# elvis-sik/muscle_synergies

Measured on NVIDIA B200. Metric: vicon_csv_loader_throughput, higher is better.
Workload: dtype f64

## Files before the change

include/ms_b200.h:

```cpp
#ifndef MS_B200_H
#define MS_B200_H

#include <stdint.h>

#ifdef __cplusplus
extern "C" {
#endif

#define MS_OK 0
#define MS_E_INVALID (-1)
#define MS_E_CUDA (-2)
#define MS_E_WORKSPACE (-3)
#define MS_E_NO_DEVICE (-4)

#ifndef MS_TILE_BYTES
#define MS_TILE_BYTES 49152
#endif
#define MS_MAX_ROW_BYTES 8192
#define MS_MAX_BLANK_ROWS 8
#define MS_MAX_SECTIONS 4

#define MS_SCAN_HAS_HIGH_BYTES 1u
#define MS_SCAN_BLANK_OVERFLOW 2u
#define MS_SCAN_HAS_CR 4u
// ... 105 lines not shown
    int64_t* d_stops;
    int64_t* d_offsets;
} ms_window_plan;
int ms_segment_trial(const double* d_left_fz, const double* d_right_fz, int64_t n, int32_t min_phase_size,
                     int32_t num_segments, void* d_work, int64_t* d_transitions, int32_t* d_loaded, int32_t* d_n_found,
                     const ms_window_plan* h_plans, int32_t n_plans, void* stream);

int ms_plan_phase_windows(const int64_t* d_transitions, const int32_t* d_n_found, int32_t num_segments,
                          int32_t cycles, int64_t divisor, int64_t n_rows, int32_t n_channels, int64_t* d_starts,
                          int64_t* d_stops, int64_t* d_offsets, void* stream);

int ms_cut_windows(const double* d_src, int64_t src_stride, int32_t n_channels, const int64_t* d_starts,
                   const int64_t* d_stops, const int64_t* d_out_offsets, int32_t n_windows, double* d_out,
                   int64_t max_window_len, void* stream);


int ms_channel_means(const double* d_src, int64_t stride, int32_t n_channels, int64_t n, double* d_mean, void* stream);
int ms_rms_envelope(const double* d_src, int64_t stride, int32_t n_channels, int64_t n, const double* d_mean,
                    int32_t window, double* d_out, int64_t out_stride, void* stream);
size_t ms_sosfilt_workspace_bytes(int64_t n, int32_t n_channels, int64_t padlen, int32_t zero_lag);
int ms_sosfilt(const double* d_src, int64_t stride, int32_t n_channels, int64_t n, const double* h_sos,
               int32_t n_sections, const double* h_zi, int64_t padlen, int32_t zero_lag, const double* d_mean,
               int32_t rectify, double* d_out, int64_t out_stride, void* d_work, void* stream);
int ms_time_normalize_windows(const double* d_env, int64_t stride, int32_t n_channels, const int64_t* d_starts,
                              const int64_t* d_stops, int32_t n_windows, int32_t reduce_to, int32_t normalize,
                              double* d_out, void* stream);


int32_t ms_nmf_resident_max_rows(int32_t m, int32_t kmax);
int ms_nmf_mu_batched(const float* d_X, int32_t n, int32_t m, const int32_t* h_ranks, const int32_t* h_x_index,
// ... 48 lines not shown
```

muscle_synergies_b200/_native.py:

```python
import ctypes
import os

_HERE = os.path.dirname(os.path.abspath(__file__))
LIB_PATH = os.path.join(_HERE, "libms_b200.so")

MS_TILE_BYTES = 49152
MS_MAX_ROW_BYTES = 8192
MS_MAX_BLANK_ROWS = 8
MS_MAX_SECTIONS = 4

MS_SCAN_HAS_HIGH_BYTES = 1
MS_SCAN_BLANK_OVERFLOW = 2
MS_SCAN_HAS_CR = 4

MS_ERR_NONE = 0xFFFFFFFFFFFFFFFF
MS_ERR_KIND_BAD_FLOAT = 1
MS_ERR_KIND_NON_ASCII = 2
MS_ERR_KIND_ROW_TOO_LONG = 3


class ScanSummary(ctypes.Structure):
    _fields_ = [
        ("n_bytes", ctypes.c_int64),
        ("n_rows", ctypes.c_int64),
# ... 57 lines not shown


class WindowPlan(ctypes.Structure):
    _fields_ = [
        ("divisor", ctypes.c_int64),
        ("n_rows", ctypes.c_int64),
        ("n_channels", ctypes.c_int32),
        ("cycles", ctypes.c_int32),
        ("d_starts", ctypes.c_void_p),
        ("d_stops", ctypes.c_void_p),
        ("d_offsets", ctypes.c_void_p),
    ]


MS_MAX_WINDOW_PLANS = 4


class NativeError(RuntimeError):
    pass


_lib = None


def _declare(L):
    vp, i64, i32 = ctypes.c_void_p, ctypes.c_int64, ctypes.c_int32
    sigs = {
        "ms_workspace_bytes": (i64, [i64]),
        "ms_workspace_masks_offset": (i64, [i64]),
        "ms_scan": (ctypes.c_int, [vp, i64, vp, i64, vp, vp]),
        "ms_scan_quoted": (ctypes.c_int, [vp, i64, vp, i64, vp, vp]),
        "ms_peek_after_blank": (ctypes.c_int, [vp, i64, vp, i32, vp, i32, vp, vp]),
        "ms_parse": (ctypes.c_int, [vp, i64, vp, ctypes.POINTER(Section), i32, vp, vp]),
        "ms_transitions_workspace_bytes": (i64, [i64]),
        "ms_find_transitions": (ctypes.c_int, [vp, vp, i64, i32, i32, vp, vp, vp, vp, vp]),
        "ms_segment_trial": (ctypes.c_int, [vp, vp, i64, i32, i32, vp, vp, vp, vp, ctypes.POINTER(WindowPlan), i32, vp]),
        "ms_cut_windows": (ctypes.c_int, [vp, i64, i32, vp, vp, vp, i32, vp, i64, vp]),
        "ms_plan_phase_windows": (ctypes.c_int, [vp, vp, i32, i32, i64, i64, i32, vp, vp, vp, vp]),
        "ms_channel_means": (ctypes.c_int, [vp, i64, i32, i64, vp, vp]),
        "ms_rms_envelope": (ctypes.c_int, [vp, i64, i32, i64, vp, i32, vp, i64, vp]),
        "ms_sosfilt_workspace_bytes": (ctypes.c_size_t, [i64, i32, i64, i32]),
        "ms_sosfilt": (ctypes.c_int, [vp, i64, i32, i64, ctypes.POINTER(ctypes.c_double), i32,
                                      ctypes.POINTER(ctypes.c_double), i64, i32, vp, i32, vp, i64, vp, vp]),
        "ms_time_normalize_windows": (ctypes.c_int, [vp, i64, i32, vp, vp, i32, i32, i32, vp, vp]),
        "ms_nmf_resident_max_rows": (i32, [i32, i32]),
        "ms_nmf_mu_batched": (ctypes.c_int, [vp, i32, i32, ctypes.POINTER(i32), ctypes.POINTER(i32), i32, vp, vp, i32,
                                             ctypes.c_float, i32, vp, vp, vp, vp, vp]),
        "ms_host_copy_stream": (ctypes.c_int, [vp, vp, i64]),
        "ms_nmf_plan": (i32, [i32, i32, ctypes.POINTER(i32), ctypes.POINTER(i32), i32, vp]),
        "ms_nmf_mu_batched_planned": (ctypes.c_int, [vp, i32, i32, vp, i32, i32, vp, vp, i32, ctypes.c_float, i32, vp, vp, vp, vp]),
        "ms_nmf_stream_workspace_bytes": (i64, [i32, i32]),
        "ms_nmf_mu_stream": (ctypes.c_int, [vp, i64, i32, ctypes.POINTER(i32), ctypes.POINTER(i32), i32, vp, vp, i32,
# ... 73 lines not shown
```

muscle_synergies_b200/csrc/ms_common.cuh:

```cuda
#pragma once
#include <cuda_runtime.h>
#include <stdint.h>

#include "../../include/ms_b200.h"

extern int64_t g_ms_launches;
extern thread_local char g_ms_last_error[256];

#define MS_CUDA_CHECK(expr)                                                                    \
    do {                                                                                       \
        cudaError_t _e = (expr);                                                               \
        if (_e != cudaSuccess) {                                                               \
            snprintf(g_ms_last_error, sizeof g_ms_last_error, "%s: %s", #expr, cudaGetErrorString(_e)); \
            return MS_E_CUDA;                                                                  \
        }                                                                                      \
    } while (0)

#define MS_COUNT_LAUNCH() ((void)__atomic_fetch_add(&g_ms_launches, 1, __ATOMIC_RELAXED))

__device__ __forceinline__ uint32_t ms_eq_flags(uint32_t w, uint32_t rep) {
    uint32_t y = w ^ rep;
    uint32_t t = (y & 0x7f7f7f7fu) + 0x7f7f7f7fu;
    return ~(t | y | 0x7f7f7f7fu);
}
// ... 50 lines not shown
```

muscle_synergies_b200/csrc/ms_fused.cu:

```cuda
#include <stdio.h>

#include "ms_field.cuh"

#ifndef FUSED_THREADS
#define FUSED_THREADS 512
#endif
#ifndef FUSED_AB_BASE
#ifndef FUSED_EARLY_COMMAS
#define FUSED_LATE_COMMAS
#endif
#define FUSED_WALK64
#define FUSED_PIN_LUT
#endif
#define FUSED_WARPS (FUSED_THREADS / 32)
#ifndef FUSED_MAX_TILE
#define FUSED_MAX_TILE MS_TILE_BYTES
#endif
#ifndef FUSED_MIN_CTAS
#define FUSED_MIN_CTAS 3
#endif
#define FUSED_MAX_REGION (FUSED_MAX_TILE + MS_MAX_ROW_BYTES)
#define FUSED_MAX_NSEG (FUSED_MAX_REGION / 16)
#define FUSED_PAD 16
#ifndef FUSED_LB_WINDOWS
// ... 933 lines not shown
static int ms_fused_tile_bytes(int32_t tile_bytes, int overhang) {
    const int largest = FUSED_MAX_REGION - overhang;
    if (tile_bytes <= 0) return largest;
    int t = tile_bytes / 16 * 16;
    if (t < 4096) t = 4096;
    if (t > largest) t = largest;
    return t;
}

extern "C" int64_t ms_load_workspace_bytes(int64_t n_bytes, int32_t tile_bytes) {
    (void)tile_bytes;
    const int64_t n_tiles = n_bytes <= 0 ? 0 : (n_bytes + 4095) / 4096;
    return FUSED_LB_OFFSET + (n_tiles + 1) * 8;
}

extern "C" int ms_load_fused(const uint8_t* d_bytes, int64_t n_bytes, const ms_load_plan* h_plan, void* d_workspace,
                             int64_t workspace_bytes, ms_load_result* d_result, uint8_t* d_peek, void* stream) {
    if (!d_bytes || !h_plan || !d_workspace || !d_result || !d_peek || n_bytes < 0) return MS_E_INVALID;
    if (((uintptr_t)d_bytes & 15) != 0 || ((uintptr_t)d_workspace & 15) != 0) return MS_E_INVALID;
    if (!h_plan->d_arena || h_plan->arena_elems < 0 || h_plan->cap_rows[0] <= 0 || h_plan->cap_rows[1] < 0) return MS_E_INVALID;
    const int overhang = ms_fused_overhang(h_plan->overhang_bytes);
    const int tile = ms_fused_tile_bytes(h_plan->tile_bytes, overhang);
    if (workspace_bytes < ms_load_workspace_bytes(n_bytes, tile)) return MS_E_WORKSPACE;
    cudaStream_t st = (cudaStream_t)stream;
    const int64_t need = FUSED_LB_OFFSET + ((n_bytes + tile - 1) / tile + 1) * 8;
    MS_CUDA_CHECK(cudaMemsetAsync(d_workspace, 0, (size_t)need, st));
    MS_CUDA_CHECK(cudaMemsetAsync(d_result, 0, sizeof(ms_load_result), st));
    MS_CUDA_CHECK(cudaMemsetAsync(&d_result->status, 0xFF, sizeof(uint64_t), st));
    const int64_t n_tiles = n_bytes == 0 ? 0 : (n_bytes + tile - 1) / tile;
    if (n_tiles == 0) return MS_OK;
// ... 16 lines not shown
```

muscle_synergies_b200/csrc/ms_segment.cu:

```cuda
#include <stdio.h>

#include <string.h>

#include "ms_common.cuh"

#define SEG_THREADS 1024
#define SEG_WARPS (SEG_THREADS / 32)
#define SEG_SPB 4
#define SEG_BLOCK_WORDS (32 * SEG_SPB)
static_assert(SEG_WARPS == 32, "a warp per bitmap word of a stretch");
#define SEG_MAX_HALO 2048

extern "C" int64_t ms_transitions_workspace_bytes(int64_t n) { return 2 * ((n + 31) / 32 + 2) * 4 + 16 + ((n + 1023) / 1024 + SEG_SPB) * 8; }

struct MsPlansArg {
    ms_window_plan p[MS_MAX_WINDOW_PLANS];
    int n;
};

__device__ void ms_plan_windows(const int64_t* __restrict__ transitions, int found, int num_segments, const ms_window_plan& pl) {
    const int per_trecho = pl.cycles ? 2 : 8, span = pl.cycles ? 4 : 1, n_windows = 4 * per_trecho;
    const bool ok = found >= num_segments && num_segments >= 40;
    int64_t off = 0;
    for (int w = 0; w < n_windows; w++) {
        int64_t a = 0, b = 0;
// ... 48 lines not shown
    if (e) {
        f = ((x >> (__ffs(e) - 1)) & 1u) ? 1u : 2u;
        l = ((x >> (31 - __clz(e))) & 1u) ? 1u : 2u;
    }
    uint32_t cy = f == 2u ? 1u : 0u;
    unsigned long long inc = seg_pack((unsigned long long)__popc(seg_changes(x, y, cy)), f, l);
#pragma unroll
    for (int d = 1; d < 32; d <<= 1) {
        const unsigned long long o = __shfl_up_sync(0xffffffffu, inc, d);
        if (lane >= d) inc = seg_combine(o, inc);
    }
    *inclusive = inc;
    return __shfl_sync(0xffffffffu, inc, 31);
}

__global__ void __launch_bounds__(SEG_THREADS, 2)
    ms_segment_kernel(const double* __restrict__ left, const double* __restrict__ right, int64_t n, int min_phase, int halo,
                      uint32_t* __restrict__ valid1, uint32_t* __restrict__ valid2, unsigned int* __restrict__ counter,
                      unsigned long long* __restrict__ summary, long long num_segments, int64_t* __restrict__ transitions,
                      int32_t* __restrict__ loaded, int32_t* __restrict__ n_found, const MsPlansArg plans) {
    extern __shared__ uint32_t s_r[];
    __shared__ bool s_last;
    __shared__ uint32_t s_v[2][SEG_BLOCK_WORDS];
    __shared__ unsigned long long s_scan[SEG_WARPS];
    __shared__ unsigned long long s_total;
    const int tid = threadIdx.x, lane = tid & 31, warp = tid >> 5;
    const int64_t n_words = (n + 31) / 32;
    const int64_t w_blk = (int64_t)blockIdx.x * SEG_BLOCK_WORDS;
    if (halo >= 0) {
        uint32_t* r1 = s_r;
        uint32_t* r2 = s_r + SEG_BLOCK_WORDS + halo;
        for (int wi0 = warp; wi0 < SEG_BLOCK_WORDS + halo; wi0 += SEG_WARPS * SEG_SPB) {
            double lv[SEG_SPB], rv[SEG_SPB];
#pragma unroll
            for (int q = 0; q < SEG_SPB; q++) {
                const int64_t i = (w_blk + wi0 + q * SEG_WARPS) * 32 + lane;
                const bool in = wi0 + q * SEG_WARPS < SEG_BLOCK_WORDS + halo && i < n;
                lv[q] = in ? left[i] : 0.0;
                rv[q] = in ? right[i] : 0.0;
            }
#pragma unroll
            for (int q = 0; q < SEG_SPB; q++) {
                const int wi = wi0 + q * SEG_WARPS;
                const int64_t i = (w_blk + wi) * 32 + lane;
                const bool a = lv[q] != 0.0, b = rv[q] != 0.0;
                const bool x1 = i < n ? a != b : true, x2 = i < n ? a && b : true;
                const uint32_t b1 = __ballot_sync(0xffffffffu, x1), b2 = __ballot_sync(0xffffffffu, x2);
                if (lane == 0 && wi < SEG_BLOCK_WORDS + halo) {
                    r1[wi] = b1;
                    r2[wi] = b2;
                }
            }
        }
        __syncthreads();
    }
#pragma unroll
    for (int q = 0; q < SEG_SPB; q++) {
        const int wl = warp + q * SEG_WARPS;
        const int64_t i_own = (w_blk + wl) * 32 + lane;
        bool v1 = false, v2 = false;
        if (i_own < n) {
            if (halo < 0) {
                const int64_t end = min(n, i_own + (int64_t)min_phase);
                v1 = v2 = true;
                for (int64_t j = i_own; j < end; j++) {
                    const bool a = left[j] != 0.0, b = right[j] != 0.0;
                    v1 = v1 && (a != b);
                    v2 = v2 && (a && b);
                    if (!v1 && !v2) break;
                }
            } else if (min_phase <= 0) {
                v1 = (s_r[wl] >> lane) & 1u;
                v2 = (s_r[SEG_BLOCK_WORDS + halo + wl] >> lane) & 1u;
            } else {
                v1 = ms_bits_all_set(s_r, wl, lane, min_phase);
                v2 = ms_bits_all_set(s_r + SEG_BLOCK_WORDS + halo, wl, lane, min_phase);
            }
        }
        const uint32_t w1 = __ballot_sync(0xffffffffu, v1), w2 = __ballot_sync(0xffffffffu, v2);
        if (lane == 0) {
            s_v[0][wl] = w1;
            s_v[1][wl] = w2;
            if (w_blk + wl < n_words) {
                valid1[w_blk + wl] = w1;
                valid2[w_blk + wl] = w2;
            }
        }
    }
    __syncthreads();
    if (warp < SEG_SPB) {
        unsigned long long inc;
        const unsigned long long total = seg_warp_scan(s_v[0][warp * 32 + lane], s_v[1][warp * 32 + lane], lane, &inc);
        if (lane == 0) summary[(int64_t)blockIdx.x * SEG_SPB + warp] = total;
    }
#if defined(SEG_ABLATE) && SEG_ABLATE == 1
    return;
#endif
    __threadfence();
    __syncthreads();
    if (tid == 0) s_last = atomicInc(counter, gridDim.x - 1) == gridDim.x - 1;
    __syncthreads();
    if (!s_last) return;
#if defined(SEG_ABLATE) && SEG_ABLATE == 2
    return;
#endif
    __threadfence();
    unsigned long long before = seg_pack(0, 2, 2);
    const int64_t n_blocks = (int64_t)gridDim.x * SEG_SPB;
    for (int64_t base = 0; base < n_blocks; base += SEG_THREADS) {
        const int64_t blk = base + tid;
        const unsigned long long mine = blk < n_blocks ? __ldcg(summary + blk) : 0ull;
        unsigned long long inc = mine;
#pragma unroll
        for (int d = 1; d < 32; d <<= 1) {
            const unsigned long long o = __shfl_up_sync(0xffffffffu, inc, d);
            if (lane >= d) inc = seg_combine(o, inc);
        }
        if (lane == 31) s_scan[warp] = inc;
        __syncthreads();
        if (warp == 0) {
            unsigned long long v = s_scan[lane];
#pragma unroll
            for (int d = 1; d < 32; d <<= 1) {
                const unsigned long long o = __shfl_up_sync(0xffffffffu, v, d);
                if (lane >= d) v = seg_combine(o, v);
            }
            s_scan[lane] = v;
            if (lane == 31) s_total = seg_combine(before, v);
        }
        __syncthreads();
        unsigned long long pre = before;
        if (warp > 0) pre = seg_combine(pre, s_scan[warp - 1]);
        {
            const unsigned long long o = __shfl_up_sync(0xffffffffu, inc, 1);
            if (lane > 0) pre = seg_combine(pre, o);
        }
        const uint32_t f = (uint32_t)(mine >> 2) & 3u;
        const bool again = (mine >> 4) + ((f && (pre & 3u) != f) ? 1u : 0u) != 0 && (long long)(pre >> 4) < num_segments;
        uint32_t todo = __ballot_sync(0xffffffffu, again);
        while (todo) {
            const int src = __ffs(todo) - 1;
            todo &= todo - 1u;
// ... 15 lines not shown
                ch &= ch - 1u;
                const int64_t hit = w * 32 + b;
                transitions[rank] = hit;
                rank++;
            }
        }
        before = s_total;
        __syncthreads();
        if ((long long)(before >> 4) >= num_segments) break;
    }
    const long long total = (long long)(before >> 4);
    const int found = (int)(total < num_segments ? total : num_segments);
    if (tid == 0) *n_found = found;
    __syncthreads();
    if (loaded)
        for (int t = tid; t < found; t += SEG_THREADS) {
            const int64_t hit = transitions[t];
            loaded[t] = (left[hit] != 0.0 ? 1 : 0) | (right[hit] != 0.0 ? 2 : 0);
        }
    if (tid < plans.n) ms_plan_windows(transitions, found, (int)(num_segments > 0x7fffffff ? 0x7fffffff : num_segments), plans.p[tid]);
}

extern "C" int ms_segment_trial(const double* d_left_fz, const double* d_right_fz, int64_t n, int32_t min_phase_size,
                                int32_t num_segments, void* d_work, int64_t* d_transitions, int32_t* d_loaded,
                                int32_t* d_n_found, const ms_window_plan* h_plans, int32_t n_plans, void* stream) {
    if (!d_left_fz || !d_right_fz || !d_work || !d_transitions || !d_n_found || n < 0 || num_segments < 0)
        return MS_E_INVALID;
    if (n_plans < 0 || n_plans > MS_MAX_WINDOW_PLANS || (n_plans > 0 && !h_plans)) return MS_E_INVALID;
    MsPlansArg plans;
    memset(&plans, 0, sizeof plans);
    for (int i = 0; i < n_plans; i++) {
        const ms_window_plan& p = h_plans[i];
        if (!p.d_starts || !p.d_stops || !p.d_offsets || p.divisor < 1 || p.n_rows < 0 || p.n_channels < 0) return MS_E_INVALID;
        plans.p[plans.n++] = p;
    }
    cudaStream_t st = (cudaStream_t)stream;
    uint32_t* v1 = (uint32_t*)d_work;
    uint32_t* v2 = v1 + ((n + 31) / 32 + 1);
    unsigned int* counter = (unsigned int*)(v2 + ((n + 31) / 32 + 1));
    unsigned long long* summary = (unsigned long long*)(((uintptr_t)(counter + 1) + 15) & ~(uintptr_t)15);
    MS_CUDA_CHECK(cudaMemsetAsync(counter, 0, sizeof(unsigned int), st));
    const int64_t n_words = (n + 31) / 32;
    const unsigned blocks = (unsigned)(n_words > 0 ? (n_words + SEG_BLOCK_WORDS - 1) / SEG_BLOCK_WORDS : 1);
    int halo = min_phase_size > 1 ? (int)(((int64_t)min_phase_size + 30) / 32) : 0;
    if (halo > SEG_MAX_HALO) halo = -1;
    const size_t smem = halo >= 0 ? sizeof(uint32_t) * 2 * (SEG_BLOCK_WORDS + halo) : 0;
    ms_segment_kernel<<<blocks, SEG_THREADS, smem, st>>>(d_left_fz, d_right_fz, n, min_phase_size, halo, v1, v2, counter, summary,
                                                         (long long)num_segments, d_transitions, d_loaded, d_n_found, plans);
    MS_COUNT_LAUNCH();
    MS_CUDA_CHECK(cudaGetLastError());
    return MS_OK;
}

extern "C" int ms_find_transitions(const double* d_left_fz, const double* d_right_fz, int64_t n, int32_t min_phase_size,
                                   int32_t num_segments, void* d_work, int64_t* d_transitions, int32_t* d_loaded,
                                   int32_t* d_n_found, void* stream) {
    return ms_segment_trial(d_left_fz, d_right_fz, n, min_phase_size, num_segments, d_work, d_transitions, d_loaded,
                            d_n_found, nullptr, 0, stream);
}

__global__ void __launch_bounds__(256)
    ms_cut_windows_kernel(const double* __restrict__ src, int64_t src_stride, int n_channels,
                          const int64_t* __restrict__ starts, const int64_t* __restrict__ stops,
                          const int64_t* __restrict__ out_offsets, double* __restrict__ out) {
    const int w = blockIdx.x / n_channels, c = blockIdx.x % n_channels;
    const int64_t a = starts[w], b = stops[w];
    const int64_t len = b > a ? b - a : 0;
    const double* __restrict__ s = src + (int64_t)c * src_stride + a;
    double* __restrict__ d = out + out_offsets[w] + (int64_t)c * len;
    for (int64_t i = (int64_t)blockIdx.y * blockDim.x + threadIdx.x; i < len; i += (int64_t)gridDim.y * blockDim.x)
        d[i] = s[i];
}

extern "C" int ms_cut_windows(const double* d_src, int64_t src_stride, int32_t n_channels, const int64_t* d_starts,
                              const int64_t* d_stops, const int64_t* d_out_offsets, int32_t n_windows, double* d_out,
                              int64_t max_window_len, void* stream) {
    if (n_windows == 0 || n_channels == 0) return MS_OK;
    if (!d_src || !d_starts || !d_stops || !d_out_offsets || !d_out || n_windows < 0 || n_channels < 0)
        return MS_E_INVALID;
    cudaStream_t st = (cudaStream_t)stream;
    unsigned gy = (unsigned)((max_window_len + 256 * 8 - 1) / (256 * 8));
    if (gy < 1) gy = 1;
    if (gy > 64) gy = 64;
    dim3 grid((unsigned)n_windows * (unsigned)n_channels, gy);
    ms_cut_windows_kernel<<<grid, 256, 0, st>>>(d_src, src_stride, n_channels, d_starts, d_stops, d_out_offsets, d_out);
    MS_COUNT_LAUNCH();
    MS_CUDA_CHECK(cudaGetLastError());
    return MS_OK;
}

__global__ void ms_plan_phase_windows_kernel(const int64_t* __restrict__ transitions, const int32_t* __restrict__ n_found,
                                             int num_segments, int cycles, int64_t divisor, int64_t n_rows, int n_channels,
                                             int64_t* __restrict__ starts, int64_t* __restrict__ stops,
                                             int64_t* __restrict__ offsets) {
    if (threadIdx.x != 0 || blockIdx.x != 0) return;
    const int per_trecho = cycles ? 2 : 8, span = cycles ? 4 : 1, n_windows = 4 * per_trecho;
    const bool ok = *n_found >= num_segments && num_segments >= 40;
    int64_t off = 0;
    for (int w = 0; w < n_windows; w++) {
        int64_t a = 0, b = 0;
        if (ok) {
            const int j = 10 * (w / per_trecho) + 1 + (w % per_trecho) * span;
            a = transitions[j] / divisor;
// ... 27 lines not shown
```

muscle_synergies_b200/segment.py:

```python
import ctypes
import os
import threading
from collections import OrderedDict
from enum import Enum, auto
from typing import List, Mapping, Optional, Sequence, Tuple, Union

from . import _native as nat
from .vicon_data.data_model import DeviceData, FrameSubfr, ViconNexusData
from .vicon_data.definitions import DeviceType


class Phase(Enum):
    DAA = "DAA"
    AS = "AS"
    DAE = "DAE"
    BL = "BL"

    @staticmethod
    def from_str(phase: str) -> "Phase":
        return {"DAA": Phase.DAA, "DAE": Phase.DAE, "AS": Phase.AS, "BL": Phase.BL}[phase.upper()]


class Trecho(Enum):
    FIRST = auto()
# ... 11 lines not shown
PhaseRef = Union[Phase, int, str]


def reactions(vicon_nexus_data: ViconNexusData):
    left_fp, right_fp = vicon_nexus_data.forcepl
    return left_fp.df["Fz"], right_fp.df["Fz"]


def _fz_tensor(dev: DeviceData):
    coords = list(dev._coords)
    if coords.count("Fz") != 1:
        raise KeyError("Fz")
    return dev.tensor[coords.index("Fz")]


_pinned_pool = threading.local()


def _pinned_like(t):
    import torch

    n = int(t.numel())
    if not hasattr(_pinned_pool, "rings"):
        _pinned_pool.rings = {}
    ring = _pinned_pool.rings.setdefault((n, t.dtype), [[], 0])
    if len(ring[0]) < 4:
        ring[0].append(torch.empty(n, dtype=t.dtype, pin_memory=True))
        return ring[0][-1]
    ring[1] = (ring[1] + 1) % len(ring[0])
    return ring[0][ring[1]]


class _TransitionSearch:

    @nat.on_tensor_device
    def __init__(self, left_fz, right_fz, min_phase_size: int, num_segments: int, extra_words: int = 0, plans=()):
        import torch

        lib = nat.lib()
        if not (left_fz.is_cuda and right_fz.is_cuda):
            raise nat.NativeError("transition_indices needs CUDA tensors; there is no CPU fallback")
        left_fz = left_fz.contiguous()
        right_fz = right_fz.contiguous()
        if left_fz.dtype != torch.float64 or right_fz.dtype != torch.float64 or left_fz.shape != right_fz.shape:
            raise ValueError("left/right reactions must be float64 vectors of equal length")
        n = int(left_fz.numel())
        dev = left_fz.device
        self.min_phase_size, self.num_segments = min_phase_size, num_segments
        self.want = want = num_segments if num_segments > 0 else max(1, n)
        work = torch.empty(int(lib.ms_transitions_workspace_bytes(n)), dtype=torch.uint8, device=dev)
        self.tail_words = (want + 2 + 1) // 2
        self.res = torch.empty(want + self.tail_words + extra_words, dtype=torch.int64, device=dev)
        self.d_transitions = self.res[:want]
        tail = self.res[want : want + self.tail_words].view(torch.int32)
        loaded, self.d_found = tail[:want], tail[want : want + 1]
        self.extra = self.res[want + self.tail_words :]
        self.stream = torch.cuda.current_stream(dev)
        plans = list(plans)
        c_plans = (nat.WindowPlan * max(1, len(plans)))()
        for i, (divisor, n_rows, n_ch) in enumerate(plans):
            base = self.extra.data_ptr() + 8 * i * _PLAN_WORDS
            c_plans[i] = nat.WindowPlan(int(divisor), int(n_rows), int(n_ch), 0, base, base + 8 * 32, base + 8 * 64)
        nat.check(
            lib.ms_segment_trial(
                left_fz.data_ptr(), right_fz.data_ptr(), n, int(min_phase_size), int(want), work.data_ptr(),
                self.d_transitions.data_ptr(), loaded.data_ptr(), self.d_found.data_ptr(), c_plans, len(plans),
                ctypes.c_void_p(self.stream.cuda_stream),
            ),
            "ms_segment_trial",
        )
        self._keep = (left_fz, right_fz, work)

    def finish(self):
        import torch

        want = self.want
        host = _pinned_like(self.res)
        host.copy_(self.res, non_blocking=True)
        self.stream.synchronize()
        tail = host[want : want + self.tail_words].view(torch.int32)
        k = int(tail[want].item())
        if self.num_segments > 0 and k < self.num_segments:
            legs = 1 if k % 2 == 0 else 2
            raise ValueError(
                f"no phase found with {self.min_phase_size} adjacent measurements with {legs} leg(s) with a nonzero reaction"
                f" (found {k} of {self.num_segments} transitions)"
            )
        return host[:k].tolist(), tail[:k].tolist(), host[want + self.tail_words :]


def transition_indices(left_fz, right_fz, min_phase_size: int = 10, num_segments: int = 40, with_loaded=False):
    idx, loaded_host, _ = _TransitionSearch(left_fz, right_fz, min_phase_size, num_segments).finish()
    if with_loaded:
        return idx, loaded_host
    return idx


def organize_transitions(to_framesubfr, transitions: Sequence[int], loaded: Sequence[int], to_framesubfr_many=None) -> Segments:

    def single_leg_phase_type(pos: int) -> Phase:
        flags = loaded[pos]
        if flags == 3 or flags == 0:
            raise ValueError(
# ... 41 lines not shown
    def __getitem__(self, i):
        if isinstance(i, slice):
            return [self[j] for j in range(*i.indices(len(self)))]
        if i < 0:
            i += len(self)
        if not 0 <= i < len(self):
            raise IndexError(i)
        if i not in self._views:
            self._views[i] = self._buffer[self._offsets[i] : self._offsets[i + 1]].view(
                self._n_ch, self._stops[i] - self._starts[i])
        return self._views[i]


_PLAN_WORDS = 32 + 32 + 33
VERIFY_DEVICE_PLAN = os.environ.get("MS_B200_VERIFY_PLAN") == "1"


class PendingSegmenter:

    def __init__(self, seg: "Segmenter", begun):
        self._seg, self._begun = seg, begun

    def finish(self) -> "Segmenter":
        if self._begun is not None:
            begun, self._begun = self._begun, None
            self._seg._complete(*begun)
        return self._seg


class Segmenter:

    def __init__(self, data: ViconNexusData, min_phase_size: int = 10, num_segments: int = 40, cut_phases_of=()):
        self._complete(*self._begin(data, min_phase_size, num_segments, cut_phases_of))

    @classmethod
    def begin(cls, data: ViconNexusData, min_phase_size: int = 10, num_segments: int = 40, cut_phases_of=()) -> "PendingSegmenter":
        seg = cls.__new__(cls)
        return PendingSegmenter(seg, seg._begin(data, min_phase_size, num_segments, cut_phases_of))

    def _begin(self, data: ViconNexusData, min_phase_size: int, num_segments: int, cut_phases_of):
        left_fp, right_fp = data.forcepl
        self._data = data
        precut = list(cut_phases_of)
        if precut and num_segments < 40:
            raise ValueError("cut_phases_of needs the full 40 transitions")
        in_launch = precut[: nat.MS_MAX_WINDOW_PLANS]
        search = _TransitionSearch(_fz_tensor(left_fp), _fz_tensor(right_fp), min_phase_size, num_segments,
                                   extra_words=_PLAN_WORDS * len(precut),
                                   plans=[self._plan_args(dev, left_fp) for dev in in_launch])
        queued = [self._queue_phase_cuts(search, dev, i, left_fp, planned=i < len(in_launch)) for i, dev in enumerate(precut)]
        return search, queued

    def _complete(self, search: "_TransitionSearch", queued):
        data = self._data
        left_fp = data.forcepl[0]
        try:
            self.transitions, self._loaded, extra = search.finish()
        finally:
            check = getattr(data, "check", None)
            if check is not None:
                check()
        self._plate = left_fp
        self._segments_made = None
        if len(self.transitions) >= 40:
# ... 35 lines not shown

        lib = nat.lib()
        src = dev.tensor
        n_ch, n_rows = int(src.shape[0]), int(src.shape[1])
        same_section = dev._frame_tracker.per_frame == plate._frame_tracker.per_frame
        divisor = 1 if same_section else plate._frame_tracker.num_subframes
        meta = search.extra[slot * _PLAN_WORDS : (slot + 1) * _PLAN_WORDS]
        starts, stops, offsets = meta[:32], meta[32:64], meta[64:97]
        out = torch.empty(max(1, n_ch * n_rows), dtype=torch.float64, device=src.device)
        sptr = ctypes.c_void_p(search.stream.cuda_stream)
        if not planned:
            nat.check(lib.ms_plan_phase_windows(search.d_transitions.data_ptr(), search.d_found.data_ptr(), search.want, 0,
                                                divisor, n_rows, n_ch, starts.data_ptr(), stops.data_ptr(),
                                                offsets.data_ptr(), sptr), "ms_plan_phase_windows")
        if n_ch:
            nat.check(lib.ms_cut_windows(src.data_ptr(), int(src.stride(0)), n_ch, starts.data_ptr(), stops.data_ptr(),
                                         offsets.data_ptr(), 32, out.data_ptr(), n_rows, sptr), "ms_cut_windows")
        return dev, out

    def _finish_phase_cuts(self, dev: DeviceData, out, meta):
        meta = meta.tolist()
        starts, stops, offsets = meta[:32], meta[32:64], meta[64:97]
        if VERIFY_DEVICE_PLAN:
            windows = [w[3] for w in self.all_phase_windows()]
            flat = dev.to_index_many([b for w in windows for b in (w.start, w.stop)])
            n_rows = int(dev.tensor.shape[1])
            for i in range(32):
                a = min(flat[2 * i], n_rows)
                if (starts[i], stops[i]) != (a, max(a, min(flat[2 * i + 1], n_rows))):
                    raise AssertionError("device-planned phase window differs from the host's")
        return _WindowViews(out, int(dev.tensor.shape[0]), starts, stops, offsets)

# ... 119 lines not shown
```

Baseline: 816.3.

## Add slim segment and cut kernel shapes that co-reside with the loader

Templates the segment kernel on thread count and makes it loop over chunks. A slim variant uses 128 threads and at most one block per SM, so it can run alongside the resident CSV loader kernel instead of waiting for SMs to free up. A host-side occupancy check decides whether the slim shape fits beside the loader's register, shared-memory and thread footprint, and picks slim or full automatically. The device-to-host result copy is now issued at begin time with a shared pinned-buffer pool and an event, which removes a later synchronous copy. The cost is fewer blocks doing the segmentation, and possible extra launch overhead from the occupancy queries.

```diff
diff --git a/include/ms_b200.h b/include/ms_b200.h
--- a/include/ms_b200.h
+++ b/include/ms_b200.h
@@ -143,6 +143,16 @@
                    const int64_t* d_stops, const int64_t* d_out_offsets, int32_t n_windows, double* d_out,
                    int64_t max_window_len, void* stream);
 
+#define MS_SHAPE_FULL 0
+#define MS_SHAPE_SLIM 1
+int ms_segment_trial_ex(const double* d_left_fz, const double* d_right_fz, int64_t n, int32_t min_phase_size,
+                        int32_t num_segments, void* d_work, int64_t* d_transitions, int32_t* d_loaded, int32_t* d_n_found,
+                        const ms_window_plan* h_plans, int32_t n_plans, int32_t shape, void* stream);
+int ms_cut_windows_ex(const double* d_src, int64_t src_stride, int32_t n_channels, const int64_t* d_starts,
+                      const int64_t* d_stops, const int64_t* d_out_offsets, int32_t n_windows, double* d_out,
+                      int64_t max_window_len, int32_t shape, void* stream);
+int ms_beside_loader_fits(void);
+
 
 int ms_channel_means(const double* d_src, int64_t stride, int32_t n_channels, int64_t n, double* d_mean, void* stream);
 int ms_rms_envelope(const double* d_src, int64_t stride, int32_t n_channels, int64_t n, const double* d_mean,
diff --git a/muscle_synergies_b200/_native.py b/muscle_synergies_b200/_native.py
--- a/muscle_synergies_b200/_native.py
+++ b/muscle_synergies_b200/_native.py
@@ -95,6 +95,8 @@
 
 
 MS_MAX_WINDOW_PLANS = 4
+MS_SHAPE_FULL = 0
+MS_SHAPE_SLIM = 1
 
 
 class NativeError(RuntimeError):
@@ -117,6 +119,9 @@
         "ms_find_transitions": (ctypes.c_int, [vp, vp, i64, i32, i32, vp, vp, vp, vp, vp]),
         "ms_segment_trial": (ctypes.c_int, [vp, vp, i64, i32, i32, vp, vp, vp, vp, ctypes.POINTER(WindowPlan), i32, vp]),
         "ms_cut_windows": (ctypes.c_int, [vp, i64, i32, vp, vp, vp, i32, vp, i64, vp]),
+        "ms_segment_trial_ex": (ctypes.c_int, [vp, vp, i64, i32, i32, vp, vp, vp, vp, ctypes.POINTER(WindowPlan), i32, i32, vp]),
+        "ms_cut_windows_ex": (ctypes.c_int, [vp, i64, i32, vp, vp, vp, i32, vp, i64, i32, vp]),
+        "ms_beside_loader_fits": (ctypes.c_int, []),
         "ms_plan_phase_windows": (ctypes.c_int, [vp, vp, i32, i32, i64, i64, i32, vp, vp, vp, vp]),
         "ms_channel_means": (ctypes.c_int, [vp, i64, i32, i64, vp, vp]),
         "ms_rms_envelope": (ctypes.c_int, [vp, i64, i32, i64, vp, i32, vp, i64, vp]),
diff --git a/muscle_synergies_b200/csrc/ms_common.cuh b/muscle_synergies_b200/csrc/ms_common.cuh
--- a/muscle_synergies_b200/csrc/ms_common.cuh
+++ b/muscle_synergies_b200/csrc/ms_common.cuh
@@ -6,6 +6,14 @@
 
 extern int64_t g_ms_launches;
 extern thread_local char g_ms_last_error[256];
+
+struct MsBlockFootprint {
+    int regs;
+    int threads;
+    int smem;
+    int blocks_per_sm;
+};
+int ms_load_kernel_footprint(MsBlockFootprint* f);
 
 #define MS_CUDA_CHECK(expr)                                                                    \
     do {                                                                                       \
diff --git a/muscle_synergies_b200/csrc/ms_fused.cu b/muscle_synergies_b200/csrc/ms_fused.cu
--- a/muscle_synergies_b200/csrc/ms_fused.cu
+++ b/muscle_synergies_b200/csrc/ms_fused.cu
@@ -971,6 +971,17 @@
     return FUSED_LB_OFFSET + (n_tiles + 1) * 8;
 }
 
+int ms_load_kernel_footprint(MsBlockFootprint* f) {
+    cudaFuncAttributes attr;
+    MS_CUDA_CHECK(cudaFuncSetAttribute(ms_load_kernel, cudaFuncAttributeMaxDynamicSharedMemorySize, FUSED_SMEM));
+    MS_CUDA_CHECK(cudaFuncGetAttributes(&attr, ms_load_kernel));
+    f->regs = attr.numRegs;
+    f->threads = FUSED_THREADS;
+    f->smem = (int)attr.sharedSizeBytes + FUSED_SMEM;
+    MS_CUDA_CHECK(cudaOccupancyMaxActiveBlocksPerMultiprocessor(&f->blocks_per_sm, ms_load_kernel, FUSED_THREADS, FUSED_SMEM));
+    return MS_OK;
+}
+
 extern "C" int ms_load_fused(const uint8_t* d_bytes, int64_t n_bytes, const ms_load_plan* h_plan, void* d_workspace,
                              int64_t workspace_bytes, ms_load_result* d_result, uint8_t* d_peek, void* stream) {
     if (!d_bytes || !h_plan || !d_workspace || !d_result || !d_peek || n_bytes < 0) return MS_E_INVALID;
diff --git a/muscle_synergies_b200/csrc/ms_segment.cu b/muscle_synergies_b200/csrc/ms_segment.cu
--- a/muscle_synergies_b200/csrc/ms_segment.cu
+++ b/muscle_synergies_b200/csrc/ms_segment.cu
@@ -5,10 +5,10 @@
 #include "ms_common.cuh"
 
 #define SEG_THREADS 1024
-#define SEG_WARPS (SEG_THREADS / 32)
 #define SEG_SPB 4
 #define SEG_BLOCK_WORDS (32 * SEG_SPB)
-static_assert(SEG_WARPS == 32, "a warp per bitmap word of a stretch");
+#define SEG_SLIM_THREADS 128
+#define SEG_SLIM_DYN_SMEM 2048
 #define SEG_MAX_HALO 2048
 
 extern "C" int64_t ms_transitions_workspace_bytes(int64_t n) { return 2 * ((n + 31) / 32 + 2) * 4 + 16 + ((n + 1023) / 1024 + SEG_SPB) * 8; }
@@ -87,84 +87,91 @@
     return __shfl_sync(0xffffffffu, inc, 31);
 }
 
-__global__ void __launch_bounds__(SEG_THREADS, 2)
+template <int THREADS>
+__global__ void __launch_bounds__(THREADS, 65536 / 32 / THREADS)
     ms_segment_kernel(const double* __restrict__ left, const double* __restrict__ right, int64_t n, int min_phase, int halo,
-                      uint32_t* __restrict__ valid1, uint32_t* __restrict__ valid2, unsigned int* __restrict__ counter,
-                      unsigned long long* __restrict__ summary, long long num_segments, int64_t* __restrict__ transitions,
-                      int32_t* __restrict__ loaded, int32_t* __restrict__ n_found, const MsPlansArg plans) {
+                      int64_t n_chunks, uint32_t* __restrict__ valid1, uint32_t* __restrict__ valid2,
+                      unsigned int* __restrict__ counter, unsigned long long* __restrict__ summary, long long num_segments,
+                      int64_t* __restrict__ transitions, int32_t* __restrict__ loaded, int32_t* __restrict__ n_found,
+                      const MsPlansArg plans) {
+    constexpr int WARPS = THREADS / 32;
+    static_assert(WARPS >= SEG_SPB && WARPS <= 32, "a warp per stretch summary; one warp scans the warps' totals");
     extern __shared__ uint32_t s_r[];
     __shared__ bool s_last;
     __shared__ uint32_t s_v[2][SEG_BLOCK_WORDS];
-    __shared__ unsigned long long s_scan[SEG_WARPS];
+    __shared__ unsigned long long s_scan[WARPS];
     __shared__ unsigned long long s_total;
     const int tid = threadIdx.x, lane = tid & 31, warp = tid >> 5;
     const int64_t n_words = (n + 31) / 32;
-    const int64_t w_blk = (int64_t)blockIdx.x * SEG_BLOCK_WORDS;
-    if (halo >= 0) {
-        uint32_t* r1 = s_r;
-        uint32_t* r2 = s_r + SEG_BLOCK_WORDS + halo;
-        for (int wi0 = warp; wi0 < SEG_BLOCK_WORDS + halo; wi0 += SEG_WARPS * SEG_SPB) {
-            double lv[SEG_SPB], rv[SEG_SPB];
-#pragma unroll
-            for (int q = 0; q < SEG_SPB; q++) {
-                const int64_t i = (w_blk + wi0 + q * SEG_WARPS) * 32 + lane;
-                const bool in = wi0 + q * SEG_WARPS < SEG_BLOCK_WORDS + halo && i < n;
-                lv[q] = in ? left[i] : 0.0;
-                rv[q] = in ? right[i] : 0.0;
-            }
-#pragma unroll
-            for (int q = 0; q < SEG_SPB; q++) {
-                const int wi = wi0 + q * SEG_WARPS;
-                const int64_t i = (w_blk + wi) * 32 + lane;
-                const bool a = lv[q] != 0.0, b = rv[q] != 0.0;
-                const bool x1 = i < n ? a != b : true, x2 = i < n ? a && b : true;
-                const uint32_t b1 = __ballot_sync(0xffffffffu, x1), b2 = __ballot_sync(0xffffffffu, x2);
-                if (lane == 0 && wi < SEG_BLOCK_WORDS + halo) {
-                    r1[wi] = b1;
-                    r2[wi] = b2;
+    for (int64_t chunk = blockIdx.x; chunk < n_chunks; chunk += gridDim.x) {
+        const int64_t w_blk = chunk * SEG_BLOCK_WORDS;
+        if (halo >= 0) {
+            uint32_t* r1 = s_r;
+            uint32_t* r2 = s_r + SEG_BLOCK_WORDS + halo;
+            for (int wi0 = warp; wi0 < SEG_BLOCK_WORDS + halo; wi0 += WARPS * SEG_SPB) {
+                double lv[SEG_SPB], rv[SEG_SPB];
+#pragma unroll
+                for (int q = 0; q < SEG_SPB; q++) {
+                    const int64_t i = (w_blk + wi0 + q * WARPS) * 32 + lane;
+                    const bool in = wi0 + q * WARPS < SEG_BLOCK_WORDS + halo && i < n;
+                    lv[q] = in ? left[i] : 0.0;
+                    rv[q] = in ? right[i] : 0.0;
                 }
+#pragma unroll
+                for (int q = 0; q < SEG_SPB; q++) {
+                    const int wi = wi0 + q * WARPS;
+                    const int64_t i = (w_blk + wi) * 32 + lane;
+                    const bool a = lv[q] != 0.0, b = rv[q] != 0.0;
+                    const bool x1 = i < n ? a != b : true, x2 = i < n ? a && b : true;
+                    const uint32_t b1 = __ballot_sync(0xffffffffu, x1), b2 = __ballot_sync(0xffffffffu, x2);
+                    if (lane == 0 && wi < SEG_BLOCK_WORDS + halo) {
+                        r1[wi] = b1;
+                        r2[wi] = b2;
+                    }
+                }
+            }
+            __syncthreads();
+        }
+#pragma unroll 4
+        for (int q = 0; q < SEG_BLOCK_WORDS / WARPS; q++) {
+            const int wl = warp + q * WARPS;
+            const int64_t i_own = (w_blk + wl) * 32 + lane;
+            bool v1 = false, v2 = false;
+            if (i_own < n) {
+                if (halo < 0) {
+                    const int64_t end = min(n, i_own + (int64_t)min_phase);
+                    v1 = v2 = true;
+                    for (int64_t j = i_own; j < end; j++) {
+                        const bool a = left[j] != 0.0, b = right[j] != 0.0;
+                        v1 = v1 && (a != b);
+                        v2 = v2 && (a && b);
+                        if (!v1 && !v2) break;
+                    }
+                } else if (min_phase <= 0) {
+                    v1 = (s_r[wl] >> lane) & 1u;
+                    v2 = (s_r[SEG_BLOCK_WORDS + halo + wl] >> lane) & 1u;
+                } else {
+                    v1 = ms_bits_all_set(s_r, wl, lane, min_phase);
+                    v2 = ms_bits_all_set(s_r + SEG_BLOCK_WORDS + halo, wl, lane, min_phase);
+                }
+            }
+            const uint32_t w1 = __ballot_sync(0xffffffffu, v1), w2 = __ballot_sync(0xffffffffu, v2);
+            if (lane == 0) {
+                s_v[0][wl] = w1;
+                s_v[1][wl] = w2;
+                if (w_blk + wl < n_words) {
+                    valid1[w_blk + wl] = w1;
+                    valid2[w_blk + wl] = w2;
+                }
             }
         }
         __syncthreads();
-    }
-#pragma unroll
-    for (int q = 0; q < SEG_SPB; q++) {
-        const int wl = warp + q * SEG_WARPS;
-        const int64_t i_own = (w_blk + wl) * 32 + lane;
-        bool v1 = false, v2 = false;
-        if (i_own < n) {
-            if (halo < 0) {
-                const int64_t end = min(n, i_own + (int64_t)min_phase);
-                v1 = v2 = true;
-                for (int64_t j = i_own; j < end; j++) {
-                    const bool a = left[j] != 0.0, b = right[j] != 0.0;
-                    v1 = v1 && (a != b);
-                    v2 = v2 && (a && b);
-                    if (!v1 && !v2) break;
-                }
-            } else if (min_phase <= 0) {
-                v1 = (s_r[wl] >> lane) & 1u;
-                v2 = (s_r[SEG_BLOCK_WORDS + halo + wl] >> lane) & 1u;
-            } else {
-                v1 = ms_bits_all_set(s_r, wl, lane, min_phase);
-                v2 = ms_bits_all_set(s_r + SEG_BLOCK_WORDS + halo, wl, lane, min_phase);
-            }
-        }
-        const uint32_t w1 = __ballot_sync(0xffffffffu, v1), w2 = __ballot_sync(0xffffffffu, v2);
-        if (lane == 0) {
-            s_v[0][wl] = w1;
-            s_v[1][wl] = w2;
-            if (w_blk + wl < n_words) {
-                valid1[w_blk + wl] = w1;
-                valid2[w_blk + wl] = w2;
-            }
-        }
-    }
-    __syncthreads();
-    if (warp < SEG_SPB) {
-        unsigned long long inc;
-        const unsigned long long total = seg_warp_scan(s_v[0][warp * 32 + lane], s_v[1][warp * 32 + lane], lane, &inc);
-        if (lane == 0) summary[(int64_t)blockIdx.x * SEG_SPB + warp] = total;
+        if (warp < SEG_SPB) {
+            unsigned long long inc;
+            const unsigned long long total = seg_warp_scan(s_v[0][warp * 32 + lane], s_v[1][warp * 32 + lane], lane, &inc);
+            if (lane == 0) summary[chunk * SEG_SPB + warp] = total;
+        }
+        if (chunk + gridDim.x < n_chunks) __syncthreads();
     }
 #if defined(SEG_ABLATE) && SEG_ABLATE == 1
     return;
@@ -179,8 +186,8 @@
 #endif
     __threadfence();
     unsigned long long before = seg_pack(0, 2, 2);
-    const int64_t n_blocks = (int64_t)gridDim.x * SEG_SPB;
-    for (int64_t base = 0; base < n_blocks; base += SEG_THREADS) {
+    const int64_t n_blocks = n_chunks * SEG_SPB;
+    for (int64_t base = 0; base < n_blocks; base += THREADS) {
         const int64_t blk = base + tid;
         const unsigned long long mine = blk < n_blocks ? __ldcg(summary + blk) : 0ull;
         unsigned long long inc = mine;
@@ -192,13 +199,13 @@
         if (lane == 31) s_scan[warp] = inc;
         __syncthreads();
         if (warp == 0) {
-            unsigned long long v = s_scan[lane];
+            unsigned long long v = lane < WARPS ? s_scan[lane] : 0ull;
 #pragma unroll
             for (int d = 1; d < 32; d <<= 1) {
                 const unsigned long long o = __shfl_up_sync(0xffffffffu, v, d);
                 if (lane >= d) v = seg_combine(o, v);
             }
-            s_scan[lane] = v;
+            if (lane < WARPS) s_scan[lane] = v;
             if (lane == 31) s_total = seg_combine(before, v);
         }
         __syncthreads();
@@ -244,19 +251,28 @@
     if (tid == 0) *n_found = found;
     __syncthreads();
     if (loaded)
-        for (int t = tid; t < found; t += SEG_THREADS) {
+        for (int t = tid; t < found; t += THREADS) {
             const int64_t hit = transitions[t];
             loaded[t] = (left[hit] != 0.0 ? 1 : 0) | (right[hit] != 0.0 ? 2 : 0);
         }
     if (tid < plans.n) ms_plan_windows(transitions, found, (int)(num_segments > 0x7fffffff ? 0x7fffffff : num_segments), plans.p[tid]);
 }
 
-extern "C" int ms_segment_trial(const double* d_left_fz, const double* d_right_fz, int64_t n, int32_t min_phase_size,
-                                int32_t num_segments, void* d_work, int64_t* d_transitions, int32_t* d_loaded,
-                                int32_t* d_n_found, const ms_window_plan* h_plans, int32_t n_plans, void* stream) {
+static int ms_sm_count(int* sms) {
+    int dev = 0;
+    MS_CUDA_CHECK(cudaGetDevice(&dev));
+    MS_CUDA_CHECK(cudaDeviceGetAttribute(sms, cudaDevAttrMultiProcessorCount, dev));
+    return MS_OK;
+}
+
+extern "C" int ms_segment_trial_ex(const double* d_left_fz, const double* d_right_fz, int64_t n, int32_t min_phase_size,
+                                   int32_t num_segments, void* d_work, int64_t* d_transitions, int32_t* d_loaded,
+                                   int32_t* d_n_found, const ms_window_plan* h_plans, int32_t n_plans, int32_t shape,
+                                   void* stream) {
     if (!d_left_fz || !d_right_fz || !d_work || !d_transitions || !d_n_found || n < 0 || num_segments < 0)
         return MS_E_INVALID;
     if (n_plans < 0 || n_plans > MS_MAX_WINDOW_PLANS || (n_plans > 0 && !h_plans)) return MS_E_INVALID;
+    if (shape != MS_SHAPE_FULL && shape != MS_SHAPE_SLIM) return MS_E_INVALID;
     MsPlansArg plans;
     memset(&plans, 0, sizeof plans);
     for (int i = 0; i < n_plans; i++) {
@@ -271,15 +287,34 @@
     unsigned long long* summary = (unsigned long long*)(((uintptr_t)(counter + 1) + 15) & ~(uintptr_t)15);
     MS_CUDA_CHECK(cudaMemsetAsync(counter, 0, sizeof(unsigned int), st));
     const int64_t n_words = (n + 31) / 32;
-    const unsigned blocks = (unsigned)(n_words > 0 ? (n_words + SEG_BLOCK_WORDS - 1) / SEG_BLOCK_WORDS : 1);
+    const int64_t n_chunks = n_words > 0 ? (n_words + SEG_BLOCK_WORDS - 1) / SEG_BLOCK_WORDS : 1;
     int halo = min_phase_size > 1 ? (int)(((int64_t)min_phase_size + 30) / 32) : 0;
     if (halo > SEG_MAX_HALO) halo = -1;
     const size_t smem = halo >= 0 ? sizeof(uint32_t) * 2 * (SEG_BLOCK_WORDS + halo) : 0;
-    ms_segment_kernel<<<blocks, SEG_THREADS, smem, st>>>(d_left_fz, d_right_fz, n, min_phase_size, halo, v1, v2, counter, summary,
-                                                         (long long)num_segments, d_transitions, d_loaded, d_n_found, plans);
+    if (shape == MS_SHAPE_SLIM && halo >= 0 && smem <= SEG_SLIM_DYN_SMEM) {
+        int sms = 0;
+        if (int rc = ms_sm_count(&sms)) return rc;
+        const unsigned blocks = (unsigned)(n_chunks < sms ? n_chunks : sms);
+        MS_CUDA_CHECK(cudaFuncSetAttribute(ms_segment_kernel<SEG_SLIM_THREADS>, cudaFuncAttributePreferredSharedMemoryCarveout,
+                                           cudaSharedmemCarveoutMaxShared));
+        ms_segment_kernel<SEG_SLIM_THREADS><<<blocks, SEG_SLIM_THREADS, smem, st>>>(
+            d_left_fz, d_right_fz, n, min_phase_size, halo, n_chunks, v1, v2, counter, summary, (long long)num_segments,
+            d_transitions, d_loaded, d_n_found, plans);
+    } else {
+        ms_segment_kernel<SEG_THREADS><<<(unsigned)n_chunks, SEG_THREADS, smem, st>>>(
+            d_left_fz, d_right_fz, n, min_phase_size, halo, n_chunks, v1, v2, counter, summary, (long long)num_segments,
+            d_transitions, d_loaded, d_n_found, plans);
+    }
     MS_COUNT_LAUNCH();
     MS_CUDA_CHECK(cudaGetLastError());
     return MS_OK;
+}
+
+extern "C" int ms_segment_trial(const double* d_left_fz, const double* d_right_fz, int64_t n, int32_t min_phase_size,
+                                int32_t num_segments, void* d_work, int64_t* d_transitions, int32_t* d_loaded,
+                                int32_t* d_n_found, const ms_window_plan* h_plans, int32_t n_plans, void* stream) {
+    return ms_segment_trial_ex(d_left_fz, d_right_fz, n, min_phase_size, num_segments, d_work, d_transitions, d_loaded,
+                               d_n_found, h_plans, n_plans, MS_SHAPE_FULL, stream);
 }
 
 extern "C" int ms_find_transitions(const double* d_left_fz, const double* d_right_fz, int64_t n, int32_t min_phase_size,
@@ -302,21 +337,120 @@
         d[i] = s[i];
 }
 
+#define CUT_SLIM_THREADS 128
+#define CUT_UNROLL 8
+#define CUT_CHUNK (32 * CUT_UNROLL * 4)
+__global__ void __launch_bounds__(CUT_SLIM_THREADS, 65536 / 32 / CUT_SLIM_THREADS)
+    ms_cut_windows_slim_kernel(const double* __restrict__ src, int64_t src_stride, int n_channels, int n_windows,
+                               const int64_t* __restrict__ starts, const int64_t* __restrict__ stops,
+                               const int64_t* __restrict__ out_offsets, double* __restrict__ out) {
+    const int lane = threadIdx.x & 31;
+    long long longest = 0;
+    for (int w = lane; w < n_windows; w += 32) {
+        const long long len = stops[w] - starts[w];
+        longest = len > longest ? len : longest;
+    }
+#pragma unroll
+    for (int d = 16; d > 0; d >>= 1) {
+        const long long o = __shfl_xor_sync(0xffffffffu, longest, d);
+        longest = o > longest ? o : longest;
+    }
+    const int64_t n_chunks = (longest + CUT_CHUNK - 1) / CUT_CHUNK;
+    const int n_warps = gridDim.x * (CUT_SLIM_THREADS / 32), rows = n_windows * n_channels;
+    const int gw = blockIdx.x * (CUT_SLIM_THREADS / 32) + (threadIdx.x >> 5);
+    const int step_chunk = n_warps / rows, step_row = n_warps % rows;
+    const int step_w = step_row / n_channels, step_c = step_row % n_channels;
+    int64_t chunk = gw / rows;
+    int w = gw % rows / n_channels, c = gw % rows % n_channels;
+    while (chunk < n_chunks) {
+        const int64_t a = starts[w], b = stops[w];
+        const int64_t len = b > a ? b - a : 0;
+        const int64_t i0 = chunk * CUT_CHUNK;
+        if (i0 < len) {
+            const double* __restrict__ s = src + (int64_t)c * src_stride + a;
+            double* __restrict__ d = out + out_offsets[w] + (int64_t)c * len;
+            const int64_t end = len < i0 + CUT_CHUNK ? len : i0 + CUT_CHUNK;
+            for (int64_t i = i0 + lane; i < end; i += 32 * CUT_UNROLL) {
+                double v[CUT_UNROLL];
+#pragma unroll
+                for (int u = 0; u < CUT_UNROLL; u++) v[u] = i + 32 * u < end ? s[i + 32 * u] : 0.0;
+#pragma unroll
+                for (int u = 0; u < CUT_UNROLL; u++)
+                    if (i + 32 * u < end) d[i + 32 * u] = v[u];
+            }
+        }
+        chunk += step_chunk;
+        c += step_c;
+        w += step_w;
+        if (c >= n_channels) {
+            c -= n_channels;
+            w++;
+        }
+        if (w >= n_windows) {
+            w -= n_windows;
+            chunk++;
+        }
+    }
+}
+
+extern "C" int ms_cut_windows_ex(const double* d_src, int64_t src_stride, int32_t n_channels, const int64_t* d_starts,
+                                 const int64_t* d_stops, const int64_t* d_out_offsets, int32_t n_windows, double* d_out,
+                                 int64_t max_window_len, int32_t shape, void* stream) {
+    if (shape != MS_SHAPE_FULL && shape != MS_SHAPE_SLIM) return MS_E_INVALID;
+    if (n_windows == 0 || n_channels == 0) return MS_OK;
+    if (!d_src || !d_starts || !d_stops || !d_out_offsets || !d_out || n_windows < 0 || n_channels < 0)
+        return MS_E_INVALID;
+    if ((int64_t)n_windows * n_channels > 0x7fffffff) return MS_E_INVALID;
+    cudaStream_t st = (cudaStream_t)stream;
+    if (shape == MS_SHAPE_SLIM) {
+        int sms = 0;
+        if (int rc = ms_sm_count(&sms)) return rc;
+        MS_CUDA_CHECK(cudaFuncSetAttribute(ms_cut_windows_slim_kernel, cudaFuncAttributePreferredSharedMemoryCarveout,
+                                           cudaSharedmemCarveoutMaxShared));
+        ms_cut_windows_slim_kernel<<<(unsigned)sms, CUT_SLIM_THREADS, 0, st>>>(d_src, src_stride, n_channels, n_windows,
+                                                                                d_starts, d_stops, d_out_offsets, d_out);
+    } else {
+        unsigned gy = (unsigned)((max_window_len + 256 * 8 - 1) / (256 * 8));
+        if (gy < 1) gy = 1;
+        if (gy > 64) gy = 64;
+        dim3 grid((unsigned)n_windows * (unsigned)n_channels, gy);
+        ms_cut_windows_kernel<<<grid, 256, 0, st>>>(d_src, src_stride, n_channels, d_starts, d_stops, d_out_offsets, d_out);
+    }
+    MS_COUNT_LAUNCH();
+    MS_CUDA_CHECK(cudaGetLastError());
+    return MS_OK;
+}
+
 extern "C" int ms_cut_windows(const double* d_src, int64_t src_stride, int32_t n_channels, const int64_t* d_starts,
                               const int64_t* d_stops, const int64_t* d_out_offsets, int32_t n_windows, double* d_out,
                               int64_t max_window_len, void* stream) {
-    if (n_windows == 0 || n_channels == 0) return MS_OK;
-    if (!d_src || !d_starts || !d_stops || !d_out_offsets || !d_out || n_windows < 0 || n_channels < 0)
-        return MS_E_INVALID;
-    cudaStream_t st = (cudaStream_t)stream;
-    unsigned gy = (unsigned)((max_window_len + 256 * 8 - 1) / (256 * 8));
-    if (gy < 1) gy = 1;
-    if (gy > 64) gy = 64;
-    dim3 grid((unsigned)n_windows * (unsigned)n_channels, gy);
-    ms_cut_windows_kernel<<<grid, 256, 0, st>>>(d_src, src_stride, n_channels, d_starts, d_stops, d_out_offsets, d_out);
-    MS_COUNT_LAUNCH();
-    MS_CUDA_CHECK(cudaGetLastError());
-    return MS_OK;
+    return ms_cut_windows_ex(d_src, src_stride, n_channels, d_starts, d_stops, d_out_offsets, n_windows, d_out,
+                             max_window_len, MS_SHAPE_FULL, stream);
+}
+
+extern "C" int ms_beside_loader_fits(void) {
+    int dev = 0, regs_sm = 0, smem_sm = 0, reserved = 0, threads_sm = 0;
+    MS_CUDA_CHECK(cudaGetDevice(&dev));
+    MS_CUDA_CHECK(cudaDeviceGetAttribute(&regs_sm, cudaDevAttrMaxRegistersPerMultiprocessor, dev));
+    MS_CUDA_CHECK(cudaDeviceGetAttribute(&smem_sm, cudaDevAttrMaxSharedMemoryPerMultiprocessor, dev));
+    MS_CUDA_CHECK(cudaDeviceGetAttribute(&reserved, cudaDevAttrReservedSharedMemoryPerBlock, dev));
+    MS_CUDA_CHECK(cudaDeviceGetAttribute(&threads_sm, cudaDevAttrMaxThreadsPerMultiProcessor, dev));
+    MsBlockFootprint loader;
+    if (int rc = ms_load_kernel_footprint(&loader)) return rc;
+    if (loader.blocks_per_sm < 1) return 0;
+    cudaFuncAttributes seg, cut;
+    MS_CUDA_CHECK(cudaFuncGetAttributes(&seg, ms_segment_kernel<SEG_SLIM_THREADS>));
+    MS_CUDA_CHECK(cudaFuncGetAttributes(&cut, ms_cut_windows_slim_kernel));
+    const MsBlockFootprint slim[2] = {{seg.numRegs, SEG_SLIM_THREADS, (int)seg.sharedSizeBytes + SEG_SLIM_DYN_SMEM, 1},
+                                      {cut.numRegs, CUT_SLIM_THREADS, (int)cut.sharedSizeBytes, 1}};
+    auto regs = [](const MsBlockFootprint& b) { return (int64_t)((b.regs * 32 + 255) / 256 * 256) * ((b.threads + 31) / 32); };
+    for (const MsBlockFootprint& s : slim) {
+        const int64_t k = loader.blocks_per_sm;
+        if (k * regs(loader) + regs(s) > regs_sm) return 0;
+        if (k * (loader.smem + reserved) + s.smem + reserved > smem_sm) return 0;
+        if (k * ((loader.threads + 31) / 32) + (s.threads + 31) / 32 > threads_sm / 32) return 0;
+    }
+    return 1;
 }
 
 __global__ void ms_plan_phase_windows_kernel(const int64_t* __restrict__ transitions, const int32_t* __restrict__ n_found,
diff --git a/muscle_synergies_b200/segment.py b/muscle_synergies_b200/segment.py
--- a/muscle_synergies_b200/segment.py
+++ b/muscle_synergies_b200/segment.py
@@ -49,27 +49,30 @@
     return dev.tensor[coords.index("Fz")]
 
 
-_pinned_pool = threading.local()
-
-
-def _pinned_like(t):
+_pinned_free = {}
+_pinned_lock = threading.Lock()
+
+
+def _pinned_take(t):
     import torch
 
-    n = int(t.numel())
-    if not hasattr(_pinned_pool, "rings"):
-        _pinned_pool.rings = {}
-    ring = _pinned_pool.rings.setdefault((n, t.dtype), [[], 0])
-    if len(ring[0]) < 4:
-        ring[0].append(torch.empty(n, dtype=t.dtype, pin_memory=True))
-        return ring[0][-1]
-    ring[1] = (ring[1] + 1) % len(ring[0])
-    return ring[0][ring[1]]
+    with _pinned_lock:
+        free = _pinned_free.get((int(t.numel()), t.dtype))
+        if free:
+            return free.pop()
+    return torch.empty(int(t.numel()), dtype=t.dtype, pin_memory=True)
+
+
+def _pinned_give(buf):
+    with _pinned_lock:
+        _pinned_free.setdefault((int(buf.numel()), buf.dtype), []).append(buf)
 
 
 class _TransitionSearch:
 
     @nat.on_tensor_device
-    def __init__(self, left_fz, right_fz, min_phase_size: int, num_segments: int, extra_words: int = 0, plans=()):
+    def __init__(self, left_fz, right_fz, min_phase_size: int, num_segments: int, extra_words: int = 0, plans=(),
+                 shape: int = nat.MS_SHAPE_FULL):
         import torch
 
         lib = nat.lib()
@@ -91,37 +94,51 @@
         loaded, self.d_found = tail[:want], tail[want : want + 1]
         self.extra = self.res[want + self.tail_words :]
         self.stream = torch.cuda.current_stream(dev)
+        self.shape = shape
         plans = list(plans)
         c_plans = (nat.WindowPlan * max(1, len(plans)))()
         for i, (divisor, n_rows, n_ch) in enumerate(plans):
             base = self.extra.data_ptr() + 8 * i * _PLAN_WORDS
             c_plans[i] = nat.WindowPlan(int(divisor), int(n_rows), int(n_ch), 0, base, base + 8 * 32, base + 8 * 64)
         nat.check(
-            lib.ms_segment_trial(
+            lib.ms_segment_trial_ex(
                 left_fz.data_ptr(), right_fz.data_ptr(), n, int(min_phase_size), int(want), work.data_ptr(),
-                self.d_transitions.data_ptr(), loaded.data_ptr(), self.d_found.data_ptr(), c_plans, len(plans),
+                self.d_transitions.data_ptr(), loaded.data_ptr(), self.d_found.data_ptr(), c_plans, len(plans), shape,
                 ctypes.c_void_p(self.stream.cuda_stream),
             ),
-            "ms_segment_trial",
+            "ms_segment_trial_ex",
         )
         self._keep = (left_fz, right_fz, work)
+        self.host = _pinned_take(self.res)
+        self.host.copy_(self.res, non_blocking=True)
+        self.done = None
+
+    def mark_done(self):
+        import torch
+
+        self.done = torch.cuda.Event()
+        self.done.record(self.stream)
 
     def finish(self):
         import torch
 
-        want = self.want
-        host = _pinned_like(self.res)
-        host.copy_(self.res, non_blocking=True)
-        self.stream.synchronize()
-        tail = host[want : want + self.tail_words].view(torch.int32)
-        k = int(tail[want].item())
-        if self.num_segments > 0 and k < self.num_segments:
-            legs = 1 if k % 2 == 0 else 2
-            raise ValueError(
-                f"no phase found with {self.min_phase_size} adjacent measurements with {legs} leg(s) with a nonzero reaction"
-                f" (found {k} of {self.num_segments} transitions)"
-            )
-        return host[:k].tolist(), tail[:k].tolist(), host[want + self.tail_words :]
+        want, host = self.want, self.host
+        if self.done is not None:
+            self.done.synchronize()
+        else:
+            self.stream.synchronize()
+        try:
+            tail = host[want : want + self.tail_words].view(torch.int32)
+            k = int(tail[want].item())
+            if self.num_segments > 0 and k < self.num_segments:
+                legs = 1 if k % 2 == 0 else 2
+                raise ValueError(
+                    f"no phase found with {self.min_phase_size} adjacent measurements with {legs} leg(s) with a nonzero"
+                    f" reaction (found {k} of {self.num_segments} transitions)"
+                )
+            return host[:k].tolist(), tail[:k].tolist(), host[want + self.tail_words :].clone()
+        finally:
+            _pinned_give(host)
 
 
 def transition_indices(left_fz, right_fz, min_phase_size: int = 10, num_segments: int = 40, with_loaded=False):
@@ -193,6 +210,26 @@
 
 _PLAN_WORDS = 32 + 32 + 33
 VERIFY_DEVICE_PLAN = os.environ.get("MS_B200_VERIFY_PLAN") == "1"
+BEGIN_SHAPE = os.environ.get("MS_B200_BEGIN_SHAPE", "auto")
+_fits = {}
+
+
+def _begin_shape(device) -> int:
+    if BEGIN_SHAPE == "full":
+        return nat.MS_SHAPE_FULL
+    if BEGIN_SHAPE == "slim":
+        return nat.MS_SHAPE_SLIM
+    if BEGIN_SHAPE != "auto":
+        raise ValueError(f"segment.BEGIN_SHAPE must be 'auto', 'full' or 'slim', not {BEGIN_SHAPE!r}")
+    if device.index not in _fits:
+        import torch
+
+        with torch.cuda.device(device):
+            rc = int(nat.lib().ms_beside_loader_fits())
+        if rc < 0:
+            nat.check(rc, "ms_beside_loader_fits")
+        _fits[device.index] = rc == 1
+    return nat.MS_SHAPE_SLIM if _fits[device.index] else nat.MS_SHAPE_FULL
 
 
 class PendingSegmenter:
@@ -210,14 +247,17 @@
 class Segmenter:
 
     def __init__(self, data: ViconNexusData, min_phase_size: int = 10, num_segments: int = 40, cut_phases_of=()):
-        self._complete(*self._begin(data, min_phase_size, num_segments, cut_phases_of))
+        self._complete(*self._begin(data, min_phase_size, num_segments, cut_phases_of, nat.MS_SHAPE_FULL))
 
     @classmethod
     def begin(cls, data: ViconNexusData, min_phase_size: int = 10, num_segments: int = 40, cut_phases_of=()) -> "PendingSegmenter":
         seg = cls.__new__(cls)
-        return PendingSegmenter(seg, seg._begin(data, min_phase_size, num_segments, cut_phases_of))
-
-    def _begin(self, data: ViconNexusData, min_phase_size: int, num_segments: int, cut_phases_of):
+        shape = _begin_shape(_fz_tensor(data.forcepl[0]).device)
+        begun = seg._begin(data, min_phase_size, num_segments, cut_phases_of, shape)
+        begun[0].mark_done()
+        return PendingSegmenter(seg, begun)
+
+    def _begin(self, data: ViconNexusData, min_phase_size: int, num_segments: int, cut_phases_of, shape: int):
         left_fp, right_fp = data.forcepl
         self._data = data
         precut = list(cut_phases_of)
@@ -226,7 +266,7 @@
         in_launch = precut[: nat.MS_MAX_WINDOW_PLANS]
         search = _TransitionSearch(_fz_tensor(left_fp), _fz_tensor(right_fp), min_phase_size, num_segments,
                                    extra_words=_PLAN_WORDS * len(precut),
-                                   plans=[self._plan_args(dev, left_fp) for dev in in_launch])
+                                   plans=[self._plan_args(dev, left_fp) for dev in in_launch], shape=shape)
         queued = [self._queue_phase_cuts(search, dev, i, left_fp, planned=i < len(in_launch)) for i, dev in enumerate(precut)]
         return search, queued
 
@@ -292,8 +332,9 @@
                                                 divisor, n_rows, n_ch, starts.data_ptr(), stops.data_ptr(),
                                                 offsets.data_ptr(), sptr), "ms_plan_phase_windows")
         if n_ch:
-            nat.check(lib.ms_cut_windows(src.data_ptr(), int(src.stride(0)), n_ch, starts.data_ptr(), stops.data_ptr(),
-                                         offsets.data_ptr(), 32, out.data_ptr(), n_rows, sptr), "ms_cut_windows")
+            nat.check(lib.ms_cut_windows_ex(src.data_ptr(), int(src.stride(0)), n_ch, starts.data_ptr(), stops.data_ptr(),
+                                            offsets.data_ptr(), 32, out.data_ptr(), n_rows, search.shape, sptr),
+                      "ms_cut_windows_ex")
         return dev, out
 
     def _finish_phase_cuts(self, dev: DeviceData, out, meta):
```

Measured after the change: 878.4 (median of 6 runs). 7.6% higher.
